# tsnorri/vcf2multialign

Measured on AMD Instinct MI355X. Metric: aligned A2M Gbases/sec, higher is better.
Workload: dtype u8

## Files before the change

vcf2multialign_amd/csrc/kernels.hpp:

```cpp
#pragma once

#include <hip/hip_runtime.h>
#include <stdint.h>

#ifdef V2M_CHECKED_BUILD
__device__ uint32_t v2m_lds_poison_seed;
#endif

namespace v2m {

typedef uint32_t u32;
typedef uint64_t u64;

constexpr int kWave = 64;
typedef u32 vec4u __attribute__((ext_vector_type(4)));
typedef vec4u vec4u_unaligned8 __attribute__((aligned(8)));

#ifdef V2M_CHECKED_BUILD
__device__ __forceinline__ u32 poison_hash(u32 seed, u32 wg, u32 i)
{
	u32 h = seed ^ (wg * 0x9E3779B1u) ^ (i * 0x85EBCA77u);
	h ^= h >> 15; h *= 0x2C1B3C6Du;
	h ^= h >> 12; h *= 0x297A2D39u;
	h ^= h >> 15;
// ... 864 lines not shown

__device__ __forceinline__ u64 resolve_word_exact(
	u64 const *__restrict__ paths, u64 words_per_copy, row_segments const &rs, u32 row, u32 s_begin, u32 s_end,
	edge_span const *__restrict__ spans, u64 const *__restrict__ overlappable,
	u32 wi, u64 w, u64 ovl_w, u32 *__restrict__ needs_serial, u32 max_back_words)
{
	u64 const ov = w & ovl_w;
	if (0 == ov) return w;
	int const b0 = __builtin_ctzll(ov);
	u32 sw = wi;
	int sb = 0;
	u64 fixed = ~ovl_w & ((1ULL << b0) - 1);
	if (fixed) {
		sb = 63 - __builtin_clzll(fixed);
	} else {
		u32 steps = 0;
		for (;;) {
			if (0 == sw) { sb = 0; break; }
			--sw;
			if (++steps > max_back_words) { atomicOr(&needs_serial[row], 1u); return w; }
			fixed = ~overlappable[sw];
			if (fixed) { sb = 63 - __builtin_clzll(fixed); break; }
		}
	}
	u64 out = (sw == wi) ? (w & ((1ULL << sb) - 1)) : 0;
	u32 cur = 0;
	for (u32 ww = sw; ww <= wi; ++ww) {
		u64 x = (ww == wi) ? w : load_row_word(paths, words_per_copy, rs, row, s_begin, s_end, ww);
		if (ww == sw) x &= ~((1ULL << sb) - 1);
		while (x) {
			constexpr int kBatch = 8;
			edge_span sp[kBatch];
			int bit[kBatch];
			bool has[kBatch];
#pragma unroll
			for (int k = 0; k < kBatch; ++k) {
				has[k] = 0 != x;
				bit[k] = has[k] ? __builtin_ctzll(x) : 0;
				x &= x - 1;
				sp[k] = spans[ww * 64u + bit[k]];
			}
#pragma unroll
			for (int k = 0; k < kBatch; ++k) {
				if (has[k] && sp[k].src >= cur) {
					cur = sp[k].tgt;
					if (ww == wi) out |= 1ULL << bit[k];
				}
			}
		}
	}
	return out;
}

__global__ __launch_bounds__(256) void resolve_effective_edges_kernel(
	u64 const *__restrict__ paths, u64 words_per_copy, u32 n_edges,
	row_segments rs, edge_span const *__restrict__ spans, u64 const *__restrict__ overlappable,
	u32 const *__restrict__ ovl_rank, u64 const *__restrict__ blocker_masks,
	u64 *__restrict__ eff, u32 n_words, u32 eff_words_per_row, u32 row_base, u32 word_base,
	u32 *__restrict__ queue, u32 *__restrict__ queue_counts , u32 shard_capacity, u32 *__restrict__ needs_serial, u32 max_back_words)
{
	u32 const row = blockIdx.x + row_base;
	u32 const shard = (blockIdx.y * gridDim.x + blockIdx.x) % kResolveQueueShards;
	u32 const s_begin = rs.seg_offsets[row], s_end = rs.seg_offsets[row + 1];
	u64 const tail_mask = (n_edges & 63) ? (1ULL << (n_edges & 63)) - 1 : ~0ULL;
	u64 const *row_words = nullptr;
	if (s_end - s_begin == 1) {
		u32 const copy = rs.seg_copy[s_begin];
		if (copy != 0xFFFFFFFFu) row_words = paths + (u64) copy * words_per_copy;
	} else {
		row_words = rs.assembled + (u64) row * rs.assembled_words;
	}
	u32 const w_first = word_base + blockIdx.y * kResolveWordsPerThread * blockDim.x + threadIdx.x;
	u64 w_all[kResolveWordsPerThread], ovl_all[kResolveWordsPerThread], mask_a[kResolveWordsPerThread], mask_b[kResolveWordsPerThread];
	u32 rank_all[kResolveWordsPerThread];
#pragma unroll
	for (int piece = 0; piece < kResolveWordsPerThread; ++piece) {
		u32 const wi = w_first + piece * blockDim.x;
		u32 const wc = wi < n_words ? wi : n_words - 1;
		w_all[piece] = row_words ? row_words[wc] : 0;
		ovl_all[piece] = overlappable[wc];
		rank_all[piece] = ovl_rank[wc];
		if (wi == (n_edges - 1) >> 6) w_all[piece] &= tail_mask;
	}
#pragma unroll
	for (int piece = 0; piece < kResolveWordsPerThread; ++piece) {
		u64 const ov = w_all[piece] & ovl_all[piece], ov2 = ov & (ov - 1);
		auto const entry = [&](u64 m) {
			return m ? rank_all[piece] + (u32) __builtin_popcountll(ovl_all[piece] & ((1ULL << __builtin_ctzll(m)) - 1)) : 0u;
		};
		mask_a[piece] = blocker_masks[entry(ov)];
		mask_b[piece] = blocker_masks[entry(ov2)];
	}
	int const lane = threadIdx.x & 63;
#pragma unroll
	for (int piece = 0; piece < kResolveWordsPerThread; ++piece) {
		u32 const wi = w_first + piece * blockDim.x;
		bool const in_range = wi < n_words;
		u64 const w = w_all[piece], ov = w & ovl_all[piece], ov2 = ov & (ov - 1);
		bool const hard = in_range && ov && ((w & mask_a[piece]) || (ov2 && ((w & mask_b[piece]) || (ov2 & (ov2 - 1)))));
		if (in_range && !hard) eff[(u64) row * eff_words_per_row + wi] = w;
		u64 const hard_lanes = __ballot(hard);
		if (hard_lanes) {
			u32 base = 0;
			if (0 == lane) base = atomicAdd(&queue_counts[shard], (u32) __builtin_popcountll(hard_lanes));
			base = __shfl(base, 0, kWave);
			if (hard) {
				u32 const slot = base + __builtin_amdgcn_mbcnt_hi((u32) (hard_lanes >> 32), __builtin_amdgcn_mbcnt_lo((u32) hard_lanes, 0));
				if (slot < shard_capacity) queue[(u64) shard * shard_capacity + slot] = (row - row_base) * n_words + wi;
				else eff[(u64) row * eff_words_per_row + wi] = resolve_word_exact(paths, words_per_copy, rs, row, s_begin, s_end, spans, overlappable, wi, w, ovl_all[piece], needs_serial, max_back_words);
			}
		}
	}
}

__global__ __launch_bounds__(256) void resolve_queued_words_kernel(
	u64 const *__restrict__ paths, u64 words_per_copy, u32 n_edges,
	row_segments rs, edge_span const *__restrict__ spans, u64 const *__restrict__ overlappable,
	u64 *__restrict__ eff, u32 n_words, u32 eff_words_per_row, u32 row_base,
	u32 const *__restrict__ queue, u32 const *__restrict__ queue_counts, u32 shard_capacity, u32 *__restrict__ needs_serial, u32 max_back_words)
{
	u32 const shard = blockIdx.x % kResolveQueueShards, part = blockIdx.x / kResolveQueueShards, parts = gridDim.x / kResolveQueueShards;
	u32 const n = queue_counts[shard] < shard_capacity ? queue_counts[shard] : shard_capacity;
	u64 const tail_mask = (n_edges & 63) ? (1ULL << (n_edges & 63)) - 1 : ~0ULL;
	for (u32 i = part * blockDim.x + threadIdx.x; i < n; i += parts * blockDim.x) {
		u32 const entry = queue[(u64) shard * shard_capacity + i];
		u32 const row = row_base + entry / n_words, wi = entry % n_words;
		u32 const s_begin = rs.seg_offsets[row], s_end = rs.seg_offsets[row + 1];
		u64 w = load_row_word(paths, words_per_copy, rs, row, s_begin, s_end, wi);
		if (wi == (n_edges - 1) >> 6) w &= tail_mask;
		eff[(u64) row * eff_words_per_row + wi] = resolve_word_exact(paths, words_per_copy, rs, row, s_begin, s_end, spans, overlappable, wi, w, overlappable[wi], needs_serial, max_back_words);
	}
}


__global__ __launch_bounds__(256) void resolve_rows_serial_kernel(
	u64 const *__restrict__ paths, u64 words_per_copy, u32 n_edges,
	row_segments rs, edge_span const *__restrict__ spans,
	u64 *__restrict__ eff, u64 eff_words_per_row, u32 n_rows, u32 const *__restrict__ needs_serial,
	u32 word_begin , u32 word_end)
{
	int const lane = threadIdx.x & 63;
	u32 const row = blockIdx.x * (blockDim.x >> 6) + (threadIdx.x >> 6);
	if (row >= n_rows) return;
	if (needs_serial && 0 == needs_serial[row]) return;

	u32 const s_begin = rs.seg_offsets[row], s_end = rs.seg_offsets[row + 1];
	u32 const n_words = (n_edges + 63) / 64;
	u64 *const eff_row = eff + (u64) row * eff_words_per_row;
	u32 cur = 0;

	for (u32 base = word_begin; base < word_end; base += 64) {
		u32 const wi = base + lane;
		u64 w = 0;
		if (wi < word_end) {
			w = load_row_word(paths, words_per_copy, rs, row, s_begin, s_end, wi);
			if (wi == n_words - 1 && (n_edges & 63))
				w &= (1ULL << (n_edges & 63)) - 1;
		}

		u32 lane_max = 0;
		for (u64 m = w; m; m &= m - 1) {
			u32 const e = wi * 64u + __builtin_ctzll(m);
			u32 const tgt = spans[e].tgt;
			lane_max = tgt > lane_max ? tgt : lane_max;
		}
		u32 incl = lane_max;
#pragma unroll
		for (int d = 1; d < 64; d <<= 1) {
			u32 const o = __shfl_up(incl, d, kWave);
			if (lane >= d) incl = o > incl ? o : incl;
		}
		u32 excl = __shfl_up(incl, 1, kWave);
		if (lane == 0) excl = 0;
		u32 const chunk_max = __shfl(incl, 63, kWave);

		u32 run = excl > cur ? excl : cur;
		bool uncertain = false;
		for (u64 m = w; m; m &= m - 1) {
			u32 const e = wi * 64u + __builtin_ctzll(m);
			edge_span const sp = spans[e];
			uncertain |= sp.src < run;
			run = sp.tgt > run ? sp.tgt : run;
		}

		u64 out = w;
		if (__any(uncertain)) {
			out = 0;
			u32 c = cur;
			u64 busy = __ballot(w != 0);
			while (busy) {
				int const j = __builtin_ctzll(busy);
				busy &= busy - 1;
				if (lane == j) {
					for (u64 m = w; m; m &= m - 1) {
						int const b = __builtin_ctzll(m);
						edge_span const sp = spans[wi * 64u + b];
						if (sp.src >= c) {
							out |= 1ULL << b;
							c = sp.tgt;
						}
					}
				}
				c = __shfl(c, j, kWave);
			}
			cur = c;
		} else {
			cur = chunk_max > cur ? chunk_max : cur;
		}
		if (wi < word_end)
			eff_row[wi] = out;
	}
}


struct tile_tables {
	u32 const *edge_begin;
	u32 const *cross_offsets;
	u32 const *cross_edges;
};

template <typename LabelPtr>
__device__ __forceinline__ void fill_patch_bytes(
	unsigned char *tile, u32 tile_base, u32 aln_begin, u32 label_len, LabelPtr label,
	u32 from, u32 to, u32 start, u32 step, char gap)
{
	for (u32 pos = from + start; pos < to; pos += step) {
		u32 const off = pos - aln_begin;
		tile[pos - tile_base] = (off < label_len) ? (unsigned char) label[off] : (unsigned char) gap;
	}
}

constexpr int kCandLds = 512;
constexpr int kLabelLds = 1024;
constexpr int kGroupRowsLds = 16;
constexpr int kEffWordsLds = kCandLds / 64 + 2;
constexpr int kLongQueueLds = 16;

struct cached_patch {
	unsigned short begin_rel;
	unsigned short span;
	unsigned short label_rel;
	unsigned short label_len;
};

struct patch_cache {
	cached_patch patch[kCandLds];
	u64 eff[kGroupRowsLds][kEffWordsLds];
	unsigned char labels[kLabelLds];
	u32 long_queue[kLongQueueLds];
	u32 long_count;
};

struct tile_job {
	u32 tile_base, tile_end;
	u32 cross_begin, n_cross, range_begin, n_range;
	u32 n_lds;
	u32 w0;
};

__device__ __forceinline__ void load_eff_cache(
	patch_cache &pc, tile_job const &job, u64 const *__restrict__ eff, u64 eff_words_per_row, u32 first_row, u32 n_rows, int t)
{
	if (0 == job.n_lds) return;
	u32 const nw = ((job.range_begin + job.n_lds - 1) >> 6) - job.w0 + 1;
	u32 const rows = n_rows < (u32) kGroupRowsLds ? n_rows : (u32) kGroupRowsLds;
	for (u32 i = t; i < rows * nw; i += kSpliceThreads)
		pc.eff[i / nw][i % nw] = eff[(u64) (first_row + i / nw) * eff_words_per_row + job.w0 + i % nw];
}

template <bool kWindow = false>
__device__ __forceinline__ void load_patch_cache(
	patch_cache &pc, tile_job &job, tile_tables const &tt, edge_patch const *__restrict__ patches, char const *__restrict__ labels,
	u64 const *__restrict__ eff, u64 eff_words_per_row, u32 tile, u32 row_begin, u32 n_group_rows, int t, u32 col_base = 0, u32 col_end = 0)
{
	job.tile_base = (kWindow ? col_base : 0u) + tile * (u32) kTileBytes;
	job.tile_end = (kWindow && col_end - job.tile_base < (u32) kTileBytes) ? col_end : job.tile_base + kTileBytes;
	job.cross_begin = tt.cross_offsets[tile];
	job.n_cross = tt.cross_offsets[tile + 1] - job.cross_begin;
	job.range_begin = tt.edge_begin[tile];
	job.n_range = tt.edge_begin[tile + 1] - job.range_begin;
	job.n_lds = job.n_range < (u32) kCandLds ? job.n_range : (u32) kCandLds;
	job.w0 = job.range_begin >> 6;
	if (job.n_lds) {
		u32 const label_base = patches[job.range_begin].label_begin;
		for (u32 i = t; i < job.n_lds; i += kSpliceThreads) {
			edge_patch const p = patches[job.range_begin + i];
			u32 const span = p.aln_end - p.aln_begin, rel = p.label_begin - label_base;
			cached_patch c;
			c.begin_rel = (unsigned short) (p.aln_begin - job.tile_base);
			c.span = span < 0xFFFFu ? (unsigned short) span : (unsigned short) 0xFFFF;
			bool const label_ok = rel + p.label_len <= (u32) kLabelLds;
			c.label_rel = label_ok ? (unsigned short) rel : (unsigned short) 0xFFFF;
			c.label_len = label_ok ? (unsigned short) p.label_len : (unsigned short) 0;
			pc.patch[i] = c;
		}
		edge_patch const last = patches[job.range_begin + job.n_lds - 1];
		u32 const label_span = last.label_begin + last.label_len - label_base;
		u32 const label_len = label_span < (u32) kLabelLds ? label_span : (u32) kLabelLds;
		for (u32 i = t; i < label_len; i += kSpliceThreads)
			pc.labels[i] = (unsigned char) labels[label_base + i];
	}
	load_eff_cache(pc, job, eff, eff_words_per_row, row_begin, n_group_rows, t);
	if (t == 0) pc.long_count = 0;
}

struct tile_patch {
	u32 edge;
	u32 aln_begin;
	u32 from, to;
	u32 label_len;
	u32 label_begin;
	bool in_lds;
};

__device__ __forceinline__ u32 candidate_edge(tile_job const &job, tile_tables const &tt, u32 i)
{
	return (i < job.n_cross) ? tt.cross_edges[job.cross_begin + i] : job.range_begin + (i - job.n_cross);
}

__device__ __forceinline__ bool candidate_in_lds(tile_job const &job, u32 i)
{
	return i >= job.n_cross && i - job.n_cross < job.n_lds;
}

template <bool kWindow = false>
__device__ __forceinline__ tile_patch candidate_patch(
	patch_cache const &pc, tile_job const &job, edge_patch const *__restrict__ patches, u32 i, u32 e, bool cached)
{
	u32 const tile_end = kWindow ? job.tile_end : job.tile_base + kTileBytes;
	cached_patch c{};
	if (cached) {
		c = pc.patch[i - job.n_cross];
		cached = c.span != 0xFFFF && c.label_rel != 0xFFFF;
	}
	tile_patch tp;
	tp.edge = e;
	if (cached) {
		tp.aln_begin = tp.from = job.tile_base + c.begin_rel;
		tp.to = tp.from + c.span < tile_end ? tp.from + c.span : tile_end;
		tp.label_len = c.label_len;
		tp.label_begin = c.label_rel;
		tp.in_lds = true;
	} else {
		edge_patch const p = patches[e];
		tp.aln_begin = p.aln_begin;
		tp.from = p.aln_begin > job.tile_base ? p.aln_begin : job.tile_base;
		tp.to = p.aln_end < tile_end ? p.aln_end : tile_end;
		tp.label_len = p.label_len;
		tp.label_begin = p.label_begin;
		tp.in_lds = false;
	}
	return tp;
}

__device__ __forceinline__ bool candidate_effective(
	patch_cache const &pc, tile_job const &job, tile_tables const &tt, u64 const *__restrict__ eff_row, u32 local_row, u32 i,
	u32 &e, bool &cached)
{
	cached = candidate_in_lds(job, i) && local_row < (u32) kGroupRowsLds;
	if (cached) {
		e = job.range_begin + (i - job.n_cross);
		return (pc.eff[local_row][(e >> 6) - job.w0] >> (e & 63)) & 1;
	}
	e = candidate_edge(job, tt, i);
	return (eff_row[e >> 6] >> (e & 63)) & 1;
}

template <bool kWindow, typename F>
__device__ __forceinline__ void for_each_effective_candidate(
	patch_cache const &pc, tile_job const &job, tile_tables const &tt, edge_patch const *__restrict__ patches,
	u64 const *__restrict__ eff_row, u32 local_row, int t, F &&f)
{
	u32 const n_cand = job.n_cross + job.n_range;
	for (u32 i = t; i < n_cand; i += kSpliceThreads) {
		u32 e;
		bool cached;
		if (!candidate_effective(pc, job, tt, eff_row, local_row, i, e, cached)) continue;
		f(candidate_patch<kWindow>(pc, job, patches, i, e, cached));
	}
}

template <bool kWindow = false>
__device__ __forceinline__ void patch_row_tile(
	unsigned char *buf, patch_cache &pc, tile_job const &job, tile_tables const &tt,
	edge_patch const *__restrict__ patches, char const *__restrict__ labels,
	u64 const *__restrict__ eff_row, u32 local_row, int t, char gap)
{
	u32 const tile_end = kWindow ? job.tile_end : job.tile_base + kTileBytes;
	for_each_effective_candidate<kWindow>(pc, job, tt, patches, eff_row, local_row, t, [&](tile_patch const &tp) {
		if (tp.to - tp.from > kLongPatch) {
			u32 const slot = atomicAdd(&pc.long_count, 1u);
			if (slot < (u32) kLongQueueLds) { pc.long_queue[slot] = tp.edge; return; }
		}
		if (tp.in_lds)
			fill_patch_bytes(buf, job.tile_base, tp.aln_begin, tp.label_len, pc.labels + tp.label_begin, tp.from, tp.to, 0, 1, gap);
		else
			fill_patch_bytes(buf, job.tile_base, tp.aln_begin, tp.label_len, labels + tp.label_begin, tp.from, tp.to, 0, 1, gap);
	});
	__syncthreads();

	u32 const n_long = pc.long_count < (u32) kLongQueueLds ? pc.long_count : (u32) kLongQueueLds;
	if (n_long) {
		for (u32 q = t >> 6; q < n_long; q += kSpliceThreads >> 6) {
			edge_patch const p = patches[pc.long_queue[q]];
			u32 const from = p.aln_begin > job.tile_base ? p.aln_begin : job.tile_base;
			u32 const to = p.aln_end < tile_end ? p.aln_end : tile_end;
			fill_patch_bytes(buf, job.tile_base, p.aln_begin, p.label_len, labels + p.label_begin, from, to, t & 63, 64, gap);
		}
		__syncthreads();
		if (t == 0) pc.long_count = 0;
	}
	V2M_POISON_LDS_RANGE(pc.long_queue, 0u, (u32) kLongQueueLds);
}

__device__ __forceinline__ void map_block(u32 b, u32 n_groups, u32 n_tiles, u32 tile_run, u32 &tile, u32 &group)
{
	u32 const per_super = tile_run * n_groups;
	u32 const super = b / per_super, within = b % per_super;
	u32 const t0 = super * tile_run;
	u32 const run = (n_tiles - t0 < tile_run) ? n_tiles - t0 : tile_run;
	group = within / run;
	tile = t0 + within % run;
}

template <bool kNonTemporal, bool kWindow>
__device__ __forceinline__ void splice_aligned_tiles(
	vec4u const *__restrict__ tmpl, u64 const *__restrict__ eff, u64 eff_words_per_row,
	tile_tables tt, edge_patch const *__restrict__ patches, char const *__restrict__ labels,
	char *__restrict__ out, u64 row_pitch, u32 n_rows, u32 rows_per_group, u32 n_groups, u32 n_tiles, u32 tile_run,
	u64 store_limit, char gap, u32 col_base, u32 col_end)
{
	__shared__ vec4u lds[2][kTileChunks];
	__shared__ patch_cache pc;

	int const t = threadIdx.x;
	u32 tile, group;
	map_block(blockIdx.x, n_groups, n_tiles, tile_run, tile, group);
	u32 const row_begin = group * rows_per_group;
	u32 const row_end = (row_begin + rows_per_group < n_rows) ? row_begin + rows_per_group : n_rows;
	V2M_POISON_LDS(lds);
	V2M_POISON_LDS(pc);

	vec4u pristine[kChunksPerThread];
#pragma unroll
	for (int k = 0; k < kChunksPerThread; ++k)
		pristine[k] = tmpl[(u64) tile * kTileChunks + t + kSpliceThreads * k];

	tile_job job;
	load_patch_cache<kWindow>(pc, job, tt, patches, labels, eff, eff_words_per_row, tile, row_begin, row_end - row_begin, t, col_base, col_end);
	u32 const tile_base = job.tile_base;

	for (u32 row = row_begin; row < row_end; ++row) {
		vec4u *const buf = lds[(row - row_begin) & 1];
		u32 const cached_row = (row - row_begin) % (u32) kGroupRowsLds;
		if (row != row_begin && 0 == cached_row)
			load_eff_cache(pc, job, eff, eff_words_per_row, row, row_end - row, t);
#pragma unroll
		for (int k = 0; k < kChunksPerThread; ++k)
			buf[t + kSpliceThreads * k] = pristine[k];
		__syncthreads();

		patch_row_tile<kWindow>((unsigned char *) buf, pc, job, tt, patches, labels, eff + (u64) row * eff_words_per_row, cached_row, t, gap);

		char *const dst = out + (u64) row * row_pitch + (u64) tile * kTileBytes;
#pragma unroll
		for (int k = 0; k < kChunksPerThread; ++k) {
			int const c = t + kSpliceThreads * k;
			if ((kWindow ? (u64) tile * kTileBytes : (u64) tile_base) + (u64) c * 16 < store_limit) {
				vec4u const nv = buf[c];
				if (kNonTemporal)
					__builtin_nontemporal_store(nv, (vec4u *) (dst + c * 16));
				else
					*(vec4u *) (dst + c * 16) = nv;
			}
		}
	}
}

template <bool kNonTemporal>
__global__ __launch_bounds__(kSpliceThreads) void splice_aligned_kernel(
	vec4u const *__restrict__ tmpl, u64 const *__restrict__ eff, u64 eff_words_per_row,
	tile_tables tt, edge_patch const *__restrict__ patches, char const *__restrict__ labels,
	char *__restrict__ out, u64 row_pitch, u32 n_rows, u32 rows_per_group, u32 n_groups, u32 n_tiles, u32 tile_run,
	u64 store_limit , char gap)
{
	splice_aligned_tiles<kNonTemporal, false>(tmpl, eff, eff_words_per_row, tt, patches, labels, out, row_pitch, n_rows, rows_per_group, n_groups,
		n_tiles, tile_run, store_limit, gap, 0u, 0u);
}

template <bool kNonTemporal>
__global__ __launch_bounds__(kSpliceThreads) void splice_aligned_window_kernel(
	vec4u const *__restrict__ tmpl, u64 const *__restrict__ eff, u64 eff_words_per_row,
	tile_tables tt, edge_patch const *__restrict__ patches, char const *__restrict__ labels,
	char *__restrict__ out, u64 row_pitch, u32 n_rows, u32 rows_per_group, u32 n_groups, u32 n_tiles, u32 tile_run,
	u64 store_limit, char gap, u32 col_base, u32 col_end)
{
	splice_aligned_tiles<kNonTemporal, true>(tmpl, eff, eff_words_per_row, tt, patches, labels, out, row_pitch, n_rows, rows_per_group, n_groups,
		n_tiles, tile_run, store_limit, gap, col_base, col_end);
}


__device__ __forceinline__ u32 zero_bytes_mask(u32 x)
{
	return ~(((x & 0x7F7F7F7Fu) + 0x7F7F7F7Fu) | x | 0x7F7F7F7Fu);
}

__device__ __forceinline__ u32 wave_inclusive_scan_u32(u32 v)
{
	v += (u32) __builtin_amdgcn_update_dpp(0, (int) v, 0x111, 0xf, 0xf, false);
	v += (u32) __builtin_amdgcn_update_dpp(0, (int) v, 0x112, 0xf, 0xf, false);
	v += (u32) __builtin_amdgcn_update_dpp(0, (int) v, 0x114, 0xf, 0xf, false);
	v += (u32) __builtin_amdgcn_update_dpp(0, (int) v, 0x118, 0xf, 0xf, false);
	v += (u32) __builtin_amdgcn_update_dpp(0, (int) v, 0x142, 0xa, 0xf, false);
	v += (u32) __builtin_amdgcn_update_dpp(0, (int) v, 0x143, 0xc, 0xf, false);
	return v;
}

template <int kN>
__device__ __forceinline__ void wave_inclusive_scan_u32_lockstep(u32 (&v)[kN])
{
#define V2M_SCAN_ROUND(CTRL, ROWS) \
	_Pragma("unroll") for (int k = 0; k < kN; ++k) v[k] += (u32) __builtin_amdgcn_update_dpp(0, (int) v[k], CTRL, ROWS, 0xf, false);
	V2M_SCAN_ROUND(0x111, 0xf)
	V2M_SCAN_ROUND(0x112, 0xf)
	V2M_SCAN_ROUND(0x114, 0xf)
	V2M_SCAN_ROUND(0x118, 0xf)
	V2M_SCAN_ROUND(0x142, 0xa)
	V2M_SCAN_ROUND(0x143, 0xc)
#undef V2M_SCAN_ROUND
}

__device__ __forceinline__ u64 wave_shift_left_u64(u64 v)
{
	u32 const lo = (u32) __builtin_amdgcn_update_dpp(0, (int) (u32) v, 0x130, 0xf, 0xf, true);
	u32 const hi = (u32) __builtin_amdgcn_update_dpp(0, (int) (u32) (v >> 32), 0x130, 0xf, 0xf, true);
	return (u64) hi << 32 | lo;
}

__device__ __forceinline__ u32 count_nonzero_bytes(unsigned char const *tile, u32 lo, u32 hi)
{
	u32 n = 0;
	while (lo < hi && (lo & 3)) n += tile[lo++] != 0;
	for (; lo + 4 <= hi; lo += 4)
		n += 4 - __builtin_popcount(zero_bytes_mask(*(u32 const *) (tile + lo)));
	while (lo < hi) n += tile[lo++] != 0;
	return n;
}

constexpr int kCountRowsMax = 256;
constexpr int kCandDeltaLds = 1024;

template <bool kWindow>
__device__ __forceinline__ void count_unaligned_tiles(
	vec4u const *__restrict__ tmpl0, u64 const *__restrict__ eff, u64 eff_words_per_row,
	tile_tables tt, edge_patch const *__restrict__ patches, char const *__restrict__ labels,
	u32 *__restrict__ tile_counts , u32 n_tiles,
	u32 n_rows, u32 rows_per_group, u32 n_groups, u32 tile_run, u32 col_base, u32 col_end)
{
	__shared__ vec4u lds[kTileChunks];
	__shared__ patch_cache pc;
	__shared__ int row_delta[kCountRowsMax];
	__shared__ int cand_delta[kCandDeltaLds];
	__shared__ u32 wave_sums[kSpliceThreads / 64];

	int const t = threadIdx.x;
	u32 tile, group;
	map_block(blockIdx.x, n_groups, n_tiles, tile_run, tile, group);
	u32 const row_begin = group * rows_per_group;
	u32 const row_end = (row_begin + rows_per_group < n_rows) ? row_begin + rows_per_group : n_rows;
	V2M_POISON_LDS(lds);
	V2M_POISON_LDS(pc);
	V2M_POISON_LDS(row_delta);
	V2M_POISON_LDS(cand_delta);
	V2M_POISON_LDS(wave_sums);

	u32 mine = 0;
#pragma unroll
	for (int k = 0; k < kChunksPerThread; ++k) {
		vec4u const v = tmpl0[(u64) tile * kTileChunks + t + kSpliceThreads * k];
		lds[t + kSpliceThreads * k] = v;
#pragma unroll
		for (int d = 0; d < 4; ++d)
			mine += 4 - __builtin_popcount(zero_bytes_mask(v[d]));
	}
#pragma unroll
	for (int d = 32; d >= 1; d >>= 1) mine += __shfl_down(mine, d, kWave);
	if ((t & 63) == 0) wave_sums[t >> 6] = mine;
	for (u32 r = t; r < (u32) kCountRowsMax; r += kSpliceThreads) row_delta[r] = 0;

	tile_job job;
	load_patch_cache<kWindow>(pc, job, tt, patches, labels, eff, eff_words_per_row, tile, row_begin, row_end - row_begin, t, col_base, col_end);
	__syncthreads();
	u32 tile_count = 0;
#pragma unroll
	for (int wv = 0; wv < kSpliceThreads / 64; ++wv) tile_count += wave_sums[wv];

	unsigned char const *const tile_bytes = (unsigned char const *) lds;
	auto patch_delta = [&](tile_patch const &tp) {
		u32 const label_end = tp.aln_begin + tp.label_len;
		int const label_in_tile = label_end > tp.from ? (int) ((label_end < tp.to ? label_end : tp.to) - tp.from) : 0;
		return label_in_tile - (int) count_nonzero_bytes(tile_bytes, tp.from - job.tile_base, tp.to - job.tile_base);
	};
	u32 const n_cand = job.n_cross + job.n_range;
	for (u32 i = t; i < n_cand && i < (u32) kCandDeltaLds; i += kSpliceThreads)
		cand_delta[i] = patch_delta(candidate_patch<kWindow>(pc, job, patches, i, candidate_edge(job, tt, i), candidate_in_lds(job, i)));
	__syncthreads();
	for (u32 sub = row_begin; sub < row_end; sub += kGroupRowsLds) {
		u32 const sub_end = sub + kGroupRowsLds < row_end ? sub + kGroupRowsLds : row_end;
		if (sub != row_begin) {
			asm volatile("s_waitcnt lgkmcnt(0)" ::: "memory");
			__syncthreads();
			load_eff_cache(pc, job, eff, eff_words_per_row, sub, sub_end - sub, t);
			__syncthreads();
		}
		u32 const sub_rows = sub_end - sub;
		u32 const nw = job.n_lds ? ((job.range_begin + job.n_lds - 1) >> 6) - job.w0 + 1 : 0;
		for (u32 idx = t; idx < sub_rows * nw; idx += kSpliceThreads) {
			u32 const r = idx / nw, w = idx % nw;
			u32 const first = (job.w0 + w) * 64u;
			u64 bits = pc.eff[r][w];
			if (first < job.range_begin) bits &= ~0ULL << (job.range_begin - first);
			u32 const cached_end = job.range_begin + job.n_lds;
			if (cached_end < first + 64u) bits &= (1ULL << (cached_end - first)) - 1;
			int delta = 0;
			for (; bits; bits &= bits - 1) {
				u32 const e = first + (u32) __builtin_ctzll(bits);
				u32 const i = job.n_cross + (e - job.range_begin);
				delta += i < (u32) kCandDeltaLds ? cand_delta[i] : patch_delta(candidate_patch<kWindow>(pc, job, patches, i, e, true));
			}
			if (delta) atomicAdd(&row_delta[sub - row_begin + r], delta);
		}
		u32 const n_other = n_cand - job.n_lds;
		for (u32 idx = t; idx < sub_rows * n_other; idx += kSpliceThreads) {
			u32 const r = idx / n_other, j = idx % n_other;
			u32 const i = j < job.n_cross ? j : j + job.n_lds;
			u32 const e = candidate_edge(job, tt, i);
			if (!((eff[(u64) (sub + r) * eff_words_per_row + (e >> 6)] >> (e & 63)) & 1)) continue;
			int const delta = i < (u32) kCandDeltaLds ? cand_delta[i] : patch_delta(candidate_patch<kWindow>(pc, job, patches, i, e, false));
			if (delta) atomicAdd(&row_delta[sub - row_begin + r], delta);
		}
	}
	__syncthreads();
	for (u32 r = t; r < row_end - row_begin; r += kSpliceThreads)
		tile_counts[(u64) (row_begin + r) * n_tiles + tile] = (u32) ((int) tile_count + row_delta[r]);
}

__global__ __launch_bounds__(kSpliceThreads) void count_unaligned_kernel(
	vec4u const *__restrict__ tmpl0, u64 const *__restrict__ eff, u64 eff_words_per_row,
	tile_tables tt, edge_patch const *__restrict__ patches, char const *__restrict__ labels,
	u32 *__restrict__ tile_counts , u32 n_tiles,
	u32 n_rows, u32 rows_per_group, u32 n_groups, u32 tile_run)
{
	count_unaligned_tiles<false>(tmpl0, eff, eff_words_per_row, tt, patches, labels, tile_counts, n_tiles, n_rows, rows_per_group, n_groups, tile_run, 0u, 0u);
}

__global__ __launch_bounds__(kSpliceThreads) void count_unaligned_window_kernel(
	vec4u const *__restrict__ tmpl0, u64 const *__restrict__ eff, u64 eff_words_per_row,
	tile_tables tt, edge_patch const *__restrict__ patches, char const *__restrict__ labels,
	u32 *__restrict__ tile_counts , u32 n_tiles,
	u32 n_rows, u32 rows_per_group, u32 n_groups, u32 tile_run, u32 col_base, u32 col_end)
{
	count_unaligned_tiles<true>(tmpl0, eff, eff_words_per_row, tt, patches, labels, tile_counts, n_tiles, n_rows, rows_per_group, n_groups, tile_run, col_base, col_end);
}

__device__ __forceinline__ u32 compaction_selector(u32 keep)
{
	u32 sel = 0x0c0c0c0cu, n = 0;
	for (u32 b = 0; b < 4; ++b)
		if (keep >> b & 1) { sel = (sel & ~(0xFFu << (8 * n))) | (b << (8 * n)); ++n; }
	return sel;
}

typedef unsigned short u16;
typedef u16 u16_unaligned __attribute__((aligned(1)));
typedef u32 u32_unaligned __attribute__((aligned(1)));
typedef u64 u64_unaligned __attribute__((aligned(1)));
typedef vec4u vec4u_unaligned __attribute__((aligned(1)));

#ifdef V2M_TUNING_BUILD
template <bool kNonTemporal>
__global__ __launch_bounds__(kSpliceThreads) void splice_unaligned_per_wave_kernel(
	vec4u const *__restrict__ tmpl0, u64 const *__restrict__ eff, u64 eff_words_per_row,
	tile_tables tt, edge_patch const *__restrict__ patches, char const *__restrict__ labels,
	u32 const *__restrict__ tile_offsets , u32 n_tiles,
	char *__restrict__ out, u64 row_pitch, u32 n_rows, u32 rows_per_group, u32 n_groups, u32 tile_run)
{
	__shared__ vec4u lds[kTileChunks];
	__shared__ patch_cache pc;
	__shared__ u32 wave_sums[kChunksPerThread * (kSpliceThreads / 64)];
	__shared__ u32 compact_sel[16];
	constexpr u32 kPackQueue = 24;
	__shared__ u32 pack_queue[kSpliceThreads / 64][kPackQueue];

	int const t = threadIdx.x;
	int const lane = t & 63, wave = __builtin_amdgcn_readfirstlane(t >> 6);
	if (t < 16) compact_sel[t] = compaction_selector((u32) t);
	u32 tile, group;
	map_block(blockIdx.x, n_groups, n_tiles, tile_run, tile, group);
	{
		u32 const t0 = tile / tile_run * tile_run;
		u32 const run = (n_tiles - t0 < tile_run) ? n_tiles - t0 : tile_run;
		if (0 == run % 8) { u32 const j = tile - t0; tile = t0 + (j & 7) * (run / 8) + (j >> 3); }
	}
	u32 const row_begin = group * rows_per_group;
	u32 const row_end = (row_begin + rows_per_group < n_rows) ? row_begin + rows_per_group : n_rows;

	vec4u pristine[kChunksPerThread];
#pragma unroll
	for (int k = 0; k < kChunksPerThread; ++k)
		pristine[k] = tmpl0[(u64) tile * kTileChunks + t + kSpliceThreads * k];

	tile_job job;
	load_patch_cache(pc, job, tt, patches, labels, eff, eff_words_per_row, tile, row_begin, row_end - row_begin, t);

	for (u32 row = row_begin; row < row_end; ++row) {
#pragma unroll
		for (int k = 0; k < kChunksPerThread; ++k)
			lds[t + kSpliceThreads * k] = pristine[k];
		__syncthreads();

		patch_row_tile((unsigned char *) lds, pc, job, tt, patches, labels, eff + (u64) row * eff_words_per_row, row - row_begin, t, 0);

		vec4u v[kChunksPerThread];
		u32 cnt[kChunksPerThread], incl[kChunksPerThread];
#pragma unroll
		for (int k = 0; k < kChunksPerThread; ++k) v[k] = lds[t + kSpliceThreads * k];
#pragma unroll
		for (int k = 0; k < kChunksPerThread; ++k) {
			u32 bytes = 0;
#pragma unroll
			for (int d = 0; d < 4; ++d) bytes = __builtin_amdgcn_msad_u8(v[k][d] ^ 0x01010101u, v[k][d], bytes);
			incl[k] = cnt[k] = bytes;
		}
		wave_inclusive_scan_u32_lockstep(incl);
#pragma unroll
		for (int k = 0; k < kChunksPerThread; ++k)
			if (lane == 63) wave_sums[k * (kSpliceThreads / 64) + wave] = incl[k];
		__syncthreads();

		u32 slot_end = lane < kChunksPerThread * (kSpliceThreads / 64) ? wave_sums[lane] : 0u;
		slot_end += (u32) __builtin_amdgcn_update_dpp(0, (int) slot_end, 0x111, 0xf, 0xf, false);
		slot_end += (u32) __builtin_amdgcn_update_dpp(0, (int) slot_end, 0x112, 0xf, 0xf, false);
		slot_end += (u32) __builtin_amdgcn_update_dpp(0, (int) slot_end, 0x114, 0xf, 0xf, false);
		slot_end += (u32) __builtin_amdgcn_update_dpp(0, (int) slot_end, 0x118, 0xf, 0xf, false);

		char *const dst = out + (u64) row * row_pitch + tile_offsets[(u64) row * n_tiles + tile];

		u32 offs[kChunksPerThread];
		u32 queued = 0, dense = 0;
#pragma unroll
		for (int k = 0; k < kChunksPerThread; ++k) {
			int const slot = k * (kSpliceThreads / 64) + wave;
			u32 const slot_begin = slot ? (u32) __builtin_amdgcn_readlane((int) slot_end, slot - 1) : 0u;
			u32 const c = cnt[k];
			u32 const off = slot_begin + incl[k] - c;
			offs[k] = off;
			if (16 == c) {
				if (kNonTemporal) __builtin_nontemporal_store(v[k], (vec4u_unaligned *) (dst + off));
				else *(vec4u_unaligned *) (dst + off) = v[k];
			}
			bool const partial = c - 1u < 15u;
			u64 const mask = __ballot(partial);
			u32 const n = (u32) __builtin_popcountll(mask);
			bool const fits = queued + n <= kPackQueue;
			u32 const pos = __builtin_amdgcn_mbcnt_hi((u32) (mask >> 32), __builtin_amdgcn_mbcnt_lo((u32) mask, queued));
			if (partial && pos < kPackQueue) pack_queue[wave][pos] = (u32) (t + kSpliceThreads * k) | c << 10 | off << 14;
			dense |= (n && !fits) ? 1u << k : 0u;
			queued = fits ? queued + n : queued;
		}
		u32 const pending = pack_queue[wave][lane < (int) kPackQueue ? lane : 0];
		for (u32 todo = dense | (queued ? 1u << kChunksPerThread : 0u); todo; todo &= todo - 1) {
			u32 const j = (u32) __builtin_ctz(todo);
			u32 e = pending;
			bool active = (u32) lane < queued;
			if (j < (u32) kChunksPerThread) {
				u32 const c = 0 == j ? cnt[0] : 1 == j ? cnt[1] : 2 == j ? cnt[2] : cnt[3];
// ... 305 lines not shown
```

Measured before the change: 6916.

## Split LDS-cached and global candidate loops, batch full-tile stores

Splits the candidate scan into a pass over LDS-cached patches and a separate pass over cross and uncached edges. Cached candidates that fail the cache check are recorded in a bitmask and handled afterwards. This removes the per-candidate branch between the LDS and global paths and lets each pass have its own fill specialisation. It also adds a whole-tile fast path that loads all LDS chunks before issuing unguarded stores, and an explicit s_waitcnt after the cache load. The hardcoded waitcnt immediate and the bitmask limit tie the code to specific constants.

```diff
diff --git a/vcf2multialign_amd/csrc/kernels.hpp b/vcf2multialign_amd/csrc/kernels.hpp
--- a/vcf2multialign_amd/csrc/kernels.hpp
+++ b/vcf2multialign_amd/csrc/kernels.hpp
@@ -1190,6 +1190,7 @@
 	}
 	load_eff_cache(pc, job, eff, eff_words_per_row, row_begin, n_group_rows, t);
 	if (t == 0) pc.long_count = 0;
+	__builtin_amdgcn_s_waitcnt(0x0F70);
 }
 
 struct tile_patch {
@@ -1198,7 +1199,6 @@
 	u32 from, to;
 	u32 label_len;
 	u32 label_begin;
-	bool in_lds;
 };
 
 __device__ __forceinline__ u32 candidate_edge(tile_job const &job, tile_tables const &tt, u32 i)
@@ -1209,63 +1209,72 @@
 __device__ __forceinline__ bool candidate_in_lds(tile_job const &job, u32 i)
 {
 	return i >= job.n_cross && i - job.n_cross < job.n_lds;
+}
+
+template <bool kWindow = false>
+__device__ __forceinline__ tile_patch global_tile_patch(tile_job const &job, edge_patch const *__restrict__ patches, u32 e)
+{
+	u32 const tile_end = kWindow ? job.tile_end : job.tile_base + kTileBytes;
+	edge_patch const p = patches[e];
+	tile_patch tp;
+	tp.edge = e;
+	tp.aln_begin = p.aln_begin;
+	tp.from = p.aln_begin > job.tile_base ? p.aln_begin : job.tile_base;
+	tp.to = p.aln_end < tile_end ? p.aln_end : tile_end;
+	tp.label_len = p.label_len;
+	tp.label_begin = p.label_begin;
+	return tp;
+}
+
+template <bool kWindow = false>
+__device__ __forceinline__ bool cached_tile_patch(patch_cache const &pc, tile_job const &job, u32 k, tile_patch &tp)
+{
+	u32 const tile_end = kWindow ? job.tile_end : job.tile_base + kTileBytes;
+	cached_patch const c = pc.patch[k];
+	tp.edge = job.range_begin + k;
+	tp.aln_begin = tp.from = job.tile_base + c.begin_rel;
+	tp.to = tp.from + c.span < tile_end ? tp.from + c.span : tile_end;
+	tp.label_len = c.label_len;
+	tp.label_begin = c.label_rel;
+	return c.span != 0xFFFF && c.label_rel != 0xFFFF;
 }
 
 template <bool kWindow = false>
 __device__ __forceinline__ tile_patch candidate_patch(
 	patch_cache const &pc, tile_job const &job, edge_patch const *__restrict__ patches, u32 i, u32 e, bool cached)
 {
-	u32 const tile_end = kWindow ? job.tile_end : job.tile_base + kTileBytes;
-	cached_patch c{};
-	if (cached) {
-		c = pc.patch[i - job.n_cross];
-		cached = c.span != 0xFFFF && c.label_rel != 0xFFFF;
-	}
 	tile_patch tp;
-	tp.edge = e;
-	if (cached) {
-		tp.aln_begin = tp.from = job.tile_base + c.begin_rel;
-		tp.to = tp.from + c.span < tile_end ? tp.from + c.span : tile_end;
-		tp.label_len = c.label_len;
-		tp.label_begin = c.label_rel;
-		tp.in_lds = true;
-	} else {
-		edge_patch const p = patches[e];
-		tp.aln_begin = p.aln_begin;
-		tp.from = p.aln_begin > job.tile_base ? p.aln_begin : job.tile_base;
-		tp.to = p.aln_end < tile_end ? p.aln_end : tile_end;
-		tp.label_len = p.label_len;
-		tp.label_begin = p.label_begin;
-		tp.in_lds = false;
-	}
-	return tp;
-}
-
-__device__ __forceinline__ bool candidate_effective(
-	patch_cache const &pc, tile_job const &job, tile_tables const &tt, u64 const *__restrict__ eff_row, u32 local_row, u32 i,
-	u32 &e, bool &cached)
-{
-	cached = candidate_in_lds(job, i) && local_row < (u32) kGroupRowsLds;
-	if (cached) {
-		e = job.range_begin + (i - job.n_cross);
-		return (pc.eff[local_row][(e >> 6) - job.w0] >> (e & 63)) & 1;
-	}
-	e = candidate_edge(job, tt, i);
-	return (eff_row[e >> 6] >> (e & 63)) & 1;
-}
-
-template <bool kWindow, typename F>
+	if (cached && cached_tile_patch<kWindow>(pc, job, i - job.n_cross, tp))
+		return tp;
+	return global_tile_patch<kWindow>(job, patches, e);
+}
+
+template <bool kWindow, typename FLds, typename FGlobal>
 __device__ __forceinline__ void for_each_effective_candidate(
 	patch_cache const &pc, tile_job const &job, tile_tables const &tt, edge_patch const *__restrict__ patches,
-	u64 const *__restrict__ eff_row, u32 local_row, int t, F &&f)
-{
-	u32 const n_cand = job.n_cross + job.n_range;
-	for (u32 i = t; i < n_cand; i += kSpliceThreads) {
-		u32 e;
-		bool cached;
-		if (!candidate_effective(pc, job, tt, eff_row, local_row, i, e, cached)) continue;
-		f(candidate_patch<kWindow>(pc, job, patches, i, e, cached));
-	}
+	u64 const *__restrict__ eff_row, u32 local_row, int t, FLds &&f_lds, FGlobal &&f_global)
+{
+	static_assert(kCandLds / kSpliceThreads <= 32, "deferred candidates are a bit mask");
+	u32 const n_cached = local_row < (u32) kGroupRowsLds ? job.n_lds : 0u;
+	u32 deferred = 0;
+	for (u32 k = t; k < n_cached; k += kSpliceThreads) {
+		u32 const e = job.range_begin + k;
+		if (!((pc.eff[local_row][(e >> 6) - job.w0] >> (e & 63)) & 1)) continue;
+		tile_patch tp;
+		if (cached_tile_patch<kWindow>(pc, job, k, tp))
+			f_lds(tp);
+		else
+			deferred |= 1u << (k / kSpliceThreads);
+	}
+
+	u32 const n_other = job.n_cross + job.n_range - n_cached;
+	for (u32 j = t; j < n_other; j += kSpliceThreads) {
+		u32 const e = j < job.n_cross ? tt.cross_edges[job.cross_begin + j] : job.range_begin + n_cached + (j - job.n_cross);
+		if (!((eff_row[e >> 6] >> (e & 63)) & 1)) continue;
+		f_global(global_tile_patch<kWindow>(job, patches, e));
+	}
+	for (; deferred; deferred &= deferred - 1)
+		f_global(global_tile_patch<kWindow>(job, patches, job.range_begin + t + (u32) __builtin_ctz(deferred) * kSpliceThreads));
 }
 
 template <bool kWindow = false>
@@ -1275,16 +1284,22 @@
 	u64 const *__restrict__ eff_row, u32 local_row, int t, char gap)
 {
 	u32 const tile_end = kWindow ? job.tile_end : job.tile_base + kTileBytes;
-	for_each_effective_candidate<kWindow>(pc, job, tt, patches, eff_row, local_row, t, [&](tile_patch const &tp) {
-		if (tp.to - tp.from > kLongPatch) {
-			u32 const slot = atomicAdd(&pc.long_count, 1u);
-			if (slot < (u32) kLongQueueLds) { pc.long_queue[slot] = tp.edge; return; }
-		}
-		if (tp.in_lds)
-			fill_patch_bytes(buf, job.tile_base, tp.aln_begin, tp.label_len, pc.labels + tp.label_begin, tp.from, tp.to, 0, 1, gap);
-		else
-			fill_patch_bytes(buf, job.tile_base, tp.aln_begin, tp.label_len, labels + tp.label_begin, tp.from, tp.to, 0, 1, gap);
-	});
+	auto queue_long = [&](tile_patch const &tp) {
+		if (tp.to - tp.from <= (u32) kLongPatch) return false;
+		u32 const slot = atomicAdd(&pc.long_count, 1u);
+		if (slot >= (u32) kLongQueueLds) return false;
+		pc.long_queue[slot] = tp.edge;
+		return true;
+	};
+	for_each_effective_candidate<kWindow>(pc, job, tt, patches, eff_row, local_row, t,
+		[&](tile_patch const &tp) {
+			if (!queue_long(tp))
+				fill_patch_bytes(buf, job.tile_base, tp.aln_begin, tp.label_len, pc.labels + tp.label_begin, tp.from, tp.to, 0, 1, gap);
+		},
+		[&](tile_patch const &tp) {
+			if (!queue_long(tp))
+				fill_patch_bytes(buf, job.tile_base, tp.aln_begin, tp.label_len, labels + tp.label_begin, tp.from, tp.to, 0, 1, gap);
+		});
 	__syncthreads();
 
 	u32 const n_long = pc.long_count < (u32) kLongQueueLds ? pc.long_count : (u32) kLongQueueLds;
@@ -1337,6 +1352,8 @@
 	tile_job job;
 	load_patch_cache<kWindow>(pc, job, tt, patches, labels, eff, eff_words_per_row, tile, row_begin, row_end - row_begin, t, col_base, col_end);
 	u32 const tile_base = job.tile_base;
+	u64 const tile_off = kWindow ? (u64) tile * kTileBytes : (u64) tile_base;
+	bool const whole_tile = tile_off + (u64) kTileBytes <= store_limit;
 
 	for (u32 row = row_begin; row < row_end; ++row) {
 		vec4u *const buf = lds[(row - row_begin) & 1];
@@ -1351,15 +1368,30 @@
 		patch_row_tile<kWindow>((unsigned char *) buf, pc, job, tt, patches, labels, eff + (u64) row * eff_words_per_row, cached_row, t, gap);
 
 		char *const dst = out + (u64) row * row_pitch + (u64) tile * kTileBytes;
-#pragma unroll
-		for (int k = 0; k < kChunksPerThread; ++k) {
-			int const c = t + kSpliceThreads * k;
-			if ((kWindow ? (u64) tile * kTileBytes : (u64) tile_base) + (u64) c * 16 < store_limit) {
-				vec4u const nv = buf[c];
+		if (whole_tile) {
+			vec4u nv[kChunksPerThread];
+#pragma unroll
+			for (int k = 0; k < kChunksPerThread; ++k)
+				nv[k] = buf[t + kSpliceThreads * k];
+#pragma unroll
+			for (int k = 0; k < kChunksPerThread; ++k) {
+				int const c = t + kSpliceThreads * k;
 				if (kNonTemporal)
-					__builtin_nontemporal_store(nv, (vec4u *) (dst + c * 16));
+					__builtin_nontemporal_store(nv[k], (vec4u *) (dst + c * 16));
 				else
-					*(vec4u *) (dst + c * 16) = nv;
+					*(vec4u *) (dst + c * 16) = nv[k];
+			}
+		} else {
+#pragma unroll
+			for (int k = 0; k < kChunksPerThread; ++k) {
+				int const c = t + kSpliceThreads * k;
+				if (tile_off + (u64) c * 16 < store_limit) {
+					vec4u const nv = buf[c];
+					if (kNonTemporal)
+						__builtin_nontemporal_store(nv, (vec4u *) (dst + c * 16));
+					else
+						*(vec4u *) (dst + c * 16) = nv;
+				}
 			}
 		}
 	}
```

Result: no change. 6902 (-0.2%).
